# Jason9339/Wavelet-Noise-in-ray-tracing

Hardware: AMD Instinct MI355X
Metric: Mnoise-samples/sec (3D wavelet, octave=4) (higher is better)
Workload: dtype f32; 1 GPU; 512^3 dense 3D WNoise grid, tile=128, octave=4 (configs[1]); tile=128, seed=12345, octave=4, device=AMD Radeon Graphics (gfx950:sramecc+:xnack-)

## Files before the change

### wavelet-noise-in-ray-tracing_amd/csrc/wn_wavelet_multiband.hip

```cpp
#include "wn_internal.hpp"

#include <algorithm>
#include <cmath>
#include <type_traits>

namespace {

using wn::GridArgs;

typedef float v4f __attribute__((ext_vector_type(4)));
typedef float v2f __attribute__((ext_vector_type(2)));

constexpr int kMaxNB = 5;
constexpr int kWW = 8, kPW = 4, kSW = 4;
constexpr int kWaves = kWW + kPW + kSW;
constexpr int kPasses = 2 * kPW;
constexpr int kBX = 512, kBY = 8, kBZ = 8;
constexpr int kRing = 4;
constexpr int kSlotZ = 8, kSlotX = 16;
constexpr int kMaxK = 5;
constexpr int kRRow = kPasses * 64;
constexpr int kRPlane = kBY * kRRow;
constexpr int kRingFloats = kRing * kBY * kBX;
constexpr int kBoxFloats = 6144;
constexpr int kDmaPlanes = kMaxNB;
constexpr int kDmaLanded = kBZ - 2;

struct MbBand {
    float oscale;
    float factor;
    int first_pass;
    int K;
    int box_off;
    int rowlen;
};

struct MbArgs {
    const float *coef;
    float *out;
    int n, nmask;
    GridArgs g;
    float inv_den;
    int nbx, nby, nbz;
    int all_full;
    MbBand band[kMaxNB];
    int pass_band[kPasses];
};

__device__ __forceinline__ float readlane_f(float v, int l)
{
    return __int_as_float(__builtin_amdgcn_readlane(__float_as_int(v), l));
}

template <int NB>
__global__ __launch_bounds__(64 * kWaves) void grid3d_mbp_kernel(const MbArgs a)
{
    extern __shared__ __attribute__((aligned(16))) float lds[];
    __shared__ __attribute__((aligned(16))) float s_box[kBoxFloats];
    __shared__ int s_mid[3][NB][32];
    __shared__ float s_w[3][NB][kSlotX][3];
    __shared__ float s_oscale[NB];
    __shared__ __attribute__((aligned(16))) float s_wy[NB][kMaxK][kBY];
    __shared__ float s_wz[NB][64];
    __shared__ int s_prep[NB][4];
    __shared__ int s_bandc[NB][4];

    const int tid = threadIdx.x, lane = tid & 63;
    const int wave = __builtin_amdgcn_readfirstlane(tid >> 6);
    const bool is_window = wave < kWW, is_collapse = wave >= kWW && wave < kWW + kPW;
    const GridArgs &g = a.g;
    float *const ring = lds + 2 * kRPlane;

    const int nyz = a.nby * a.nbz;
    const long long total = (long long)a.nbx * nyz;
    const int item0 = (int)(total * blockIdx.x / gridDim.x), item1 = (int)(total * (blockIdx.x + 1) / gridDim.x);
    const int nb = item1 - item0;
    if (nb <= 0) return;
    const int G = nb * kBZ;

    struct Brick { int bx, by, bz; };
    auto brick_of = [&](int item) {
        Brick k;
        k.bx = item / nyz;
        k.by = (item - k.bx * nyz) / a.nbz;
        k.bz = item - k.bx * nyz - k.by * a.nbz;
        return k;
    };
    auto advance = [&](Brick &k) {
        if (++k.bz == a.nbz) { k.bz = 0; ++k.by; }
        if (k.by == a.nby) { k.by = 0; ++k.bx; }
    };

    auto fill_tables = [&](int buf, const Brick &k) {
        int tt = tid;
        asm volatile("" : "+v"(tt));
        const int b = tt >> 5, slot = tt & 31;
        if (b < NB && slot < kSlotX + 2) {
            int idx;
            if (slot < kSlotZ) idx = min(k.by * kBY + slot, g.ny - 1);
            else if (slot < kSlotX) idx = g.z0 + min(k.bz * kBZ + slot - kSlotZ, g.nz - 1);
            else idx = (slot == kSlotX) ? k.bx * kBX : min(k.bx * kBX + kBX - 1, g.nx - 1);
            const float c = wn::lattice_coord_fast(idx, (float)g.den, a.inv_den, g.base_range, s_oscale[b], g.post_scale);
            int m;
            float w0, w1, w2;
            wn::bspline(c, m, w0, w1, w2);
            s_mid[buf][b][slot] = m;
            if (slot < kSlotX) {
                s_w[buf][b][slot][0] = w0;
                s_w[buf][b][slot][1] = w1;
                s_w[buf][b][slot][2] = w2;
            }
        }
    };
    auto sgpr = [](int v) { return __builtin_amdgcn_readfirstlane(v); };
    auto fresh_rows = [&](int b, int K, int tA, int tB, bool same_column) {
        const int d = sgpr(s_mid[tB][b][kSlotZ]) - sgpr(s_mid[tA][b][kSlotZ]);
        return (same_column && d >= 0 && d <= 2) ? d : K;
    };

    auto derive_tables = [&](int b, int tA, int tB, bool same_column, bool first) {
        const int l = lane;
        {
            const int K = s_bandc[b][0];
            const int kz0 = s_mid[tB][b][kSlotZ] - 1;
            const int kzm = (K == 4) ? (kz0 & 3) : ((kz0 + 20 * 65536) % 5);
            {
                const int zi = l >> 3, j = l & 7;
                int t0 = kzm + (s_mid[tB][b][kSlotZ + zi] - s_mid[tB][b][kSlotZ]);
                t0 -= (t0 >= K) ? K : 0;
                const float w0 = s_w[tB][b][kSlotZ + zi][0], w1 = s_w[tB][b][kSlotZ + zi][1], w2 = s_w[tB][b][kSlotZ + zi][2];
                s_wz[b][l] = j == 0 ? w0 : j == 1 ? w1 : j == 2 ? w2 : __int_as_float(t0);
            }
            if (l < kMaxK * kBY) {
                const int j = l >> 3, yi = l & 7;
                const int dd = j - (s_mid[tB][b][yi] - s_mid[tB][b][0]);
                const float w0 = s_w[tB][b][yi][0], w1 = s_w[tB][b][yi][1], w2 = s_w[tB][b][yi][2];
                float f = a.band[0].factor;
#pragma unroll
                for (int bb = 1; bb < NB; ++bb) f = (b == bb) ? a.band[bb].factor : f;
                s_wy[b][j][yi] = ((unsigned)dd <= 2u ? (dd == 0 ? w0 : dd == 1 ? w1 : w2) : 0.0f) * f;
            }
            if (l == 0) {
                const int dz = s_mid[tB][b][kSlotZ] - s_mid[tA][b][kSlotZ];
                s_prep[b][0] = kzm;
                s_prep[b][1] = (!first && same_column && dz >= 0 && dz <= 2) ? dz : K;
                s_prep[b][2] = (s_mid[tB][b][kSlotX] - 1) & 3;
            }
        }
    };

    Brick cur = brick_of(item0), nxt = cur;
    advance(nxt);
    Brick nxt2 = nxt;
    advance(nxt2);
    if (tid < NB) {
        int K = a.band[0].K, box_off = a.band[0].box_off, rowlen = a.band[0].rowlen, fp = a.band[0].first_pass;
#pragma unroll
        for (int bb = 1; bb < NB; ++bb) {
            K = (tid == bb) ? a.band[bb].K : K;
            box_off = (tid == bb) ? a.band[bb].box_off : box_off;
            rowlen = (tid == bb) ? a.band[bb].rowlen : rowlen;
            fp = (tid == bb) ? a.band[bb].first_pass : fp;
        }
        s_bandc[tid][0] = K;
        s_bandc[tid][1] = box_off;
        s_bandc[tid][2] = rowlen;
        s_bandc[tid][3] = fp;
        float os = a.band[0].oscale;
#pragma unroll
        for (int bb = 1; bb < NB; ++bb) os = (tid == bb) ? a.band[bb].oscale : os;
        s_oscale[tid] = os;
    }
    __syncthreads();
    fill_tables(0, cur);
    if (nb > 1) fill_tables(1, nxt);
    __syncthreads();
    int tb = 0, t = 0;
    auto next_brick = [&]() {
        cur = nxt;
        nxt = nxt2;
        advance(nxt2);
        tb = (tb == 2) ? 0 : tb + 1;
        ++t;
    };

    if (is_collapse) {
        struct Pass {
            int id, band, col0, box_off, rowlen;
            float factor;
        };
        Pass ps[2];
        int pk[2];
#pragma unroll
        for (int i = 0; i < 2; ++i) {
            Pass &P = ps[i];
            P.id = (wave - kWW) + kPW * i;
            P.band = sgpr(a.pass_band[P.id]);
            const int bb0 = max(P.band, 0);
            pk[i] = P.band >= 0 ? sgpr(s_bandc[bb0][0]) : 0;
            P.box_off = sgpr(s_bandc[bb0][1]);
            P.rowlen = sgpr(s_bandc[bb0][2]);
            P.col0 = 64 * (P.id - sgpr(s_bandc[bb0][3]));
            float f = a.band[0].factor;
#pragma unroll
            for (int bb = 1; bb < NB; ++bb) f = (bb0 == bb) ? a.band[bb].factor : f;
            P.factor = __int_as_float(sgpr(__float_as_int(f)));
        }
        auto prep_brick = [&](const Pass &P, auto &yc, float &wzv, auto kc) {
            constexpr int K = decltype(kc)::value;
            if constexpr (K > 0) {
                const int kzm = sgpr(s_prep[P.band][0]), d = sgpr(s_prep[P.band][1]);
                wzv = s_wz[P.band][lane];
                const float *img = s_box + P.box_off + min(sgpr(s_prep[P.band][2]) + P.col0 + lane, P.rowlen - 1);
#pragma unroll
                for (int sl = 0; sl < K; ++sl) {
                    const int tau = (sl - kzm + K) % K;
                    if (tau >= K - d) {
                        const float *row = img + (tau - (K - d)) * K * P.rowlen;
#pragma unroll
                        for (int j = 0; j < K; ++j) {
                            const float cj = row[j * P.rowlen];
                            const v2f c2 = {cj, cj};
#pragma unroll
                            for (int h = 0; h < 2; ++h) {
                                const v4f w4 = *reinterpret_cast<const v4f *>(&s_wy[P.band][j][4 * h]);
                                const v2f wlo = {w4.x, w4.y}, whi = {w4.z, w4.w};
                                yc[2 * h][sl] = (j == 0) ? wlo * c2 : __builtin_elementwise_fma(wlo, c2, yc[2 * h][sl]);
                                yc[2 * h + 1][sl] = (j == 0) ? whi * c2 : __builtin_elementwise_fma(whi, c2, yc[2 * h + 1][sl]);
                            }
                        }
                    }
                }
            }
        };
        auto p1_slice = [&](float *Rw, int zi, const auto &yc, float wzv, auto kc) {
            constexpr int K = decltype(kc)::value;
            if constexpr (K > 0) {
                const float w0 = readlane_f(wzv, zi * 8), w1 = readlane_f(wzv, zi * 8 + 1), w2 = readlane_f(wzv, zi * 8 + 2);
                const int t0 = __builtin_amdgcn_readlane(__float_as_int(wzv), zi * 8 + 3);
                auto taps = [&](auto tc) {
                    constexpr int T0 = decltype(tc)::value, T1 = (T0 + 1) % K, T2 = (T0 + 2) % K;
#pragma unroll
                    for (int p2 = 0; p2 < kBY / 2; ++p2) {
                        v2f v = v2f{w0, w0} * yc[p2][T0];
                        v = __builtin_elementwise_fma(v2f{w1, w1}, yc[p2][T1], v);
                        v = __builtin_elementwise_fma(v2f{w2, w2}, yc[p2][T2], v);
                        Rw[(2 * p2) * kRRow] = v.x;
                        Rw[(2 * p2 + 1) * kRRow] = v.y;
                    }
                };
                using std::integral_constant;
                if (t0 == 0) taps(integral_constant<int, 0>{});
                else if (t0 == 1) taps(integral_constant<int, 1>{});
                else if (t0 == 2) taps(integral_constant<int, 2>{});
                else if (t0 == 3 || K == 4) taps(integral_constant<int, 3>{});
                else taps(integral_constant<int, K - 1>{});
            }
        };
        auto collapse_role = [&](auto k0c, auto k1c) {
            constexpr int K0 = decltype(k0c)::value, K1 = decltype(k1c)::value;
            v2f yc0[kBY / 2][K0 > 0 ? K0 : 1], yc1[kBY / 2][K1 > 0 ? K1 : 1];
            float wzv0 = 0.0f, wzv1 = 0.0f;
            float *const Rw0 = lds + 64 * ps[0].id + lane, *const Rw1 = lds + 64 * ps[1].id + lane;
            wn::lds_barrier();
            prep_brick(ps[0], yc0, wzv0, k0c);
            prep_brick(ps[1], yc1, wzv1, k1c);
            p1_slice(Rw0, 0, yc0, wzv0, k0c);
            p1_slice(Rw1, 0, yc1, wzv1, k1c);
            wn::lds_barrier();
            for (int gp = 0; gp < G + 2; ++gp) {
                const int zi = gp & (kBZ - 1);
                if (gp < G) {
                    if (gp + 1 < G) {
                        if (zi == kBZ - 1) {
                            prep_brick(ps[0], yc0, wzv0, k0c);
                            prep_brick(ps[1], yc1, wzv1, k1c);
                        }
                        const int rs = ((gp + 1) & 1) * kRPlane;
                        p1_slice(Rw0 + rs, (gp + 1) & (kBZ - 1), yc0, wzv0, k0c);
                        p1_slice(Rw1 + rs, (gp + 1) & (kBZ - 1), yc1, wzv1, k1c);
                    }
                    if (zi == kBZ - 1) next_brick();
                }
                wn::lds_barrier();
            }
        };
        using std::integral_constant;
        const int k0 = pk[0], k1 = pk[1];
        if (k0 == 4 && k1 == 4) collapse_role(integral_constant<int, 4>{}, integral_constant<int, 4>{});
        else if (k0 == 4 && k1 == 5) collapse_role(integral_constant<int, 4>{}, integral_constant<int, 5>{});
        else if (k0 == 5 && k1 == 4) collapse_role(integral_constant<int, 5>{}, integral_constant<int, 4>{});
        else if (k0 == 5 && k1 == 5) collapse_role(integral_constant<int, 5>{}, integral_constant<int, 5>{});
        else if (k0 == 4) collapse_role(integral_constant<int, 4>{}, integral_constant<int, 0>{});
        else if (k0 == 5) collapse_role(integral_constant<int, 5>{}, integral_constant<int, 0>{});
        else collapse_role(integral_constant<int, 0>{}, integral_constant<int, 0>{});
    } else if (is_window) {
        const int xw = (wave >> 2) & 1, wr = wave & 3;
        float ww[NB][4][4];
        int wbase[NB];
        auto x_weights = [&](int tbuf, int bx) {
            const float den = (float)g.den;
            const int x0 = bx * kBX + xw * 256 + lane * 4;
            float xbase[4];
#pragma unroll
            for (int q = 0; q < 4; ++q) {
                const float xi = (float)min(x0 + q, g.nx - 1);
                xbase[q] = ((a.inv_den != 0.0f) ? xi * a.inv_den : xi / den) * g.base_range;
            }
#pragma unroll
            for (int b = 0; b < NB; ++b) {
                int m[4];
                float w[4][3];
#pragma unroll
                for (int q = 0; q < 4; ++q) {
                    float cc = xbase[q] * a.band[b].oscale;
                    cc = cc * g.post_scale;
                    wn::bspline(cc, m[q], w[q][0], w[q][1], w[q][2]);
                }
                wbase[b] = 64 * a.band[b].first_pass + m[0] - s_mid[tbuf][b][kSlotX];
#pragma unroll
                for (int q = 0; q < 4; ++q) {
                    const bool up = m[q] != m[0];
                    ww[b][q][0] = up ? 0.0f : w[q][0];
                    ww[b][q][1] = up ? w[q][0] : w[q][1];
                    ww[b][q][2] = up ? w[q][1] : w[q][2];
                    ww[b][q][3] = up ? w[q][2] : 0.0f;
                }
            }
        };
        auto phaseC = [&](int rslot, int ringslot) {
            float acc[2][4];
            const float *Rp = lds + rslot * kRPlane + wr * kRRow;
#pragma unroll
            for (int b = 0; b < NB; ++b) {
                float v[2][4];
#pragma unroll
                for (int h = 0; h < 2; ++h)
#pragma unroll
                    for (int i = 0; i < 4; ++i) v[h][i] = Rp[h * 4 * kRRow + wbase[b] + i];
#pragma unroll
                for (int h = 0; h < 2; ++h)
#pragma unroll
                    for (int q = 0; q < 4; ++q) {
                        float s = (b == 0) ? ww[b][q][0] * v[h][0] : __builtin_fmaf(ww[b][q][0], v[h][0], acc[h][q]);
                        s = __builtin_fmaf(ww[b][q][1], v[h][1], s);
                        s = __builtin_fmaf(ww[b][q][2], v[h][2], s);
                        s = __builtin_fmaf(ww[b][q][3], v[h][3], s);
                        acc[h][q] = s;
                    }
            }
#pragma unroll
            for (int h = 0; h < 2; ++h)
                *reinterpret_cast<v4f *>(ring + (ringslot * kBY + wr + 4 * h) * kBX + xw * 256 + lane * 4) =
                    v4f{acc[h][0], acc[h][1], acc[h][2], acc[h][3]};
        };

        x_weights(0, cur.bx);
        wn::lds_barrier();
        wn::lds_barrier();
        for (int gp = 0; gp < G + 2; ++gp) {
            const int zi = gp & (kBZ - 1);
            if (gp < G) {
                phaseC(gp & 1, gp & (kRing - 1));
                if (zi == kBZ - 1) {
                    const int tb1 = (tb == 2) ? 0 : tb + 1, tb2 = (tb1 == 2) ? 0 : tb1 + 1;
                    if (t + 2 < nb) fill_tables(tb2, nxt2);
                    if (t + 1 < nb && nxt.bx != cur.bx) x_weights(tb1, nxt.bx);
                    next_brick();
                }
            }
            wn::lds_barrier();
        }
    } else {
        const int sw = wave - (kWW + kPW);
        int bK[NB], bBox[NB], bRow[NB];
#pragma unroll
        for (int b = 0; b < NB; ++b) {
            bK[b] = sgpr(s_bandc[b][0]);
            bBox[b] = sgpr(s_bandc[b][1]);
            bRow[b] = sgpr(s_bandc[b][2]);
        }
        auto request_band = [&](auto bc, int tA, int tB, bool same_column, bool first) {
            constexpr int b = decltype(bc)::value;
            if constexpr (b < NB) {
                const int K = bK[b];
                const int d = first ? K : fresh_rows(b, K, tA, tB, same_column);
                const int jy0 = sgpr(s_mid[tB][b][0]) - 1, kz0 = sgpr(s_mid[tB][b][kSlotZ]) - 1 + (K - d);
                const int r = min(lane, K * K - 1);
                const int f = (K == 4) ? (r >> 2) : ((r * 13) >> 6);
                const int j = r - f * K;
                const int rowoff = (((kz0 + f) & a.nmask) * a.n + ((jy0 + j) & a.nmask)) * a.n;
                const int ix0 = (sgpr(s_mid[tB][b][kSlotX]) - 1) & ~3;
                const unsigned voff = (unsigned)((ix0 + 4 * lane) & a.nmask) * 4u;
                for (int rr = sw; rr < d * K; rr += kSW) {
                    const char *rowp = reinterpret_cast<const char *>(a.coef + __builtin_amdgcn_readlane(rowoff, rr));
                    if (4 * lane < bRow[b])
                        __builtin_amdgcn_global_load_lds((const __attribute__((address_space(1))) void *)(rowp + voff),
                                                         (__attribute__((address_space(3))) void *)&s_box[bBox[b] + rr * bRow[b]],
                                                         16, 0, 0);
                }
            }
        };
        Brick sb = cur;
        const size_t plane_stride = (size_t)g.ny * g.nx;
        float *orow = nullptr;
        auto brick_pointer = [&]() {
            orow = a.out + ((size_t)(sb.bz * kBZ) * g.ny + sb.by * kBY + 2 * sw) * g.nx + sb.bx * kBX + lane * 4;
        };
        brick_pointer();
        auto store_plane = [&](int p) {
            const int zi = p & (kBZ - 1), ringslot = p & (kRing - 1);
            const float *src = ring + (ringslot * kBY + 2 * sw) * kBX + lane * 4;
            v4f v[4];
#pragma unroll
            for (int q = 0; q < 4; ++q) v[q] = *reinterpret_cast<const v4f *>(src + (q >> 1) * kBX + (q & 1) * 256);
            if (a.all_full) {
#pragma unroll
                for (int q = 0; q < 4; ++q) *reinterpret_cast<v4f *>(orow + (size_t)(q >> 1) * g.nx + (q & 1) * 256) = v[q];
            } else {
                const int z = sb.bz * kBZ + zi;
#pragma unroll
                for (int q = 0; q < 4; ++q) {
                    const int row = 2 * sw + (q >> 1), xh = q & 1;
                    const int y = sb.by * kBY + row, x = sb.bx * kBX + xh * 256 + lane * 4;
                    if (y < g.ny && z < g.nz && x + 3 < g.nx)
                        *reinterpret_cast<v4f *>(orow + (size_t)(q >> 1) * g.nx + (q & 1) * 256) = v[q];
                }
            }
            orow += plane_stride;
            if (zi == kBZ - 1) {
                advance(sb);
                brick_pointer();
            }
        };

        using std::integral_constant;
        request_band(integral_constant<int, 0>{}, 0, 0, false, true);
        request_band(integral_constant<int, 1>{}, 0, 0, false, true);
        request_band(integral_constant<int, 2>{}, 0, 0, false, true);
        request_band(integral_constant<int, 3>{}, 0, 0, false, true);
        request_band(integral_constant<int, 4>{}, 0, 0, false, true);
        for (int b = sw; b < NB; b += kSW) derive_tables(b, 0, 0, false, true);
        asm volatile("s_waitcnt vmcnt(0)" ::: "memory");
        wn::lds_barrier();
        wn::lds_barrier();
        for (int gp = 0; gp < G + 2; ++gp) {
            const int zi = gp & (kBZ - 1);
            if (gp >= 2) store_plane(gp - 2);
            if (gp < G) {
                if (zi < NB && t + 1 < nb) {
                    const int tb1 = (tb == 2) ? 0 : tb + 1;
                    const bool same = nxt.bx == cur.bx && nxt.by == cur.by;
                    if (zi == 0) request_band(integral_constant<int, 0>{}, tb, tb1, same, false);
                    else if (zi == 1) request_band(integral_constant<int, 1>{}, tb, tb1, same, false);
                    else if (zi == 2) request_band(integral_constant<int, 2>{}, tb, tb1, same, false);
                    else if (zi == 3) request_band(integral_constant<int, 3>{}, tb, tb1, same, false);
                    else request_band(integral_constant<int, 4>{}, tb, tb1, same, false);
                }
                if (zi == kBZ - 2 && t + 1 < nb)
                    for (int b = sw; b < NB; b += kSW)
                        derive_tables(b, tb, (tb == 2) ? 0 : tb + 1, nxt.bx == cur.bx && nxt.by == cur.by, false);
                if (zi == kDmaLanded) {
                    if (a.all_full) asm volatile("s_waitcnt vmcnt(%0)" ::"n"(4 * (kDmaLanded - kDmaPlanes + 1)) : "memory");
                    else asm volatile("s_waitcnt vmcnt(0)" ::: "memory");
                }
                if (zi == kBZ - 1) next_brick();
            }
            wn::lds_barrier();
        }
    }
}

template <int NB>
bool launch_mbp(const MbArgs &a, size_t lds, long long bricks, hipStream_t s)
{
    const void *fn = reinterpret_cast<const void *>(&grid3d_mbp_kernel<NB>);
    if (!wn::ensure_dynamic_lds(fn, wn::current_device(), lds)) return false;
    const int cus = wn::device_compute_units(wn::current_device());
    const int grid = (int)std::min<long long>(bricks, cus);
    hipLaunchKernelGGL((grid3d_mbp_kernel<NB>), dim3(grid), dim3(64 * kWaves), lds, s, a);
    return true;
}

}

namespace wn {

int multiband_try(const wn_tile *tile, const GridArgs &g, int nbands, const float *oscale, const float *weights,
                  float out_div, float *out_dev, hipStream_t stream, int min_bricks_per_cu)
{
    if (nbands < 1 || nbands > kMaxNB || tile->n == 0 || wn::pow2_mask(tile->n) < 0) return kDeclined;
    if (g.nx <= 256 || !vec4_ok(out_dev, g.nx) || g.ny <= 0 || g.nz <= 0 || g.z_const_mode || g.z0 < 0) return kDeclined;
    MbArgs a{};
    int passes = 0, box_off = 0;
    for (int w = 0; w < kPasses; ++w) a.pass_band[w] = -1;
    for (int b = 0; b < nbands; ++b) {
        LatticeStep ls;
        if (!lattice_step(g, oscale[b], false, false, 0.0, &ls) || !ls.two_mids()) return kDeclined;
        const int K = (int)std::max<long long>(4, std::max(ls.extent(kBY), ls.extent(kBZ)));
        if (K > kMaxK) return kDeclined;
        const int ex = (int)ls.extent(kBX) + 1;
        const int np = (ex + 63) / 64;
        if (passes + np > kPasses) return kDeclined;
        a.band[b].first_pass = passes;
        for (int p = 0; p < np; ++p) a.pass_band[passes++] = b;
        a.band[b].oscale = oscale[b];
        a.band[b].factor = (float)((double)(weights ? weights[b] : 1.0f) * (double)g.out_scale / (double)out_div);
        a.band[b].K = K;
        a.band[b].rowlen = (ex + 3 + 3) & ~3;
        if (a.band[b].rowlen > 256) return kDeclined;
        a.band[b].box_off = box_off;
        box_off += K * K * a.band[b].rowlen;
    }
    if (box_off > kBoxFloats) return kDeclined;
    const size_t lds = (size_t)(2 * kRPlane + kRingFloats) * sizeof(float);
    a.coef = tile->dev;
    a.out = out_dev;
    a.n = tile->n;
    a.nmask = wn::pow2_mask(tile->n);
    a.g = g;
    a.inv_den = wn::inv_den_of(g.den);
    a.nbx = (g.nx + kBX - 1) / kBX;
    a.nby = (g.ny + kBY - 1) / kBY;
    a.nbz = (g.nz + kBZ - 1) / kBZ;
    a.all_full = (g.nx % kBX == 0 && g.ny % kBY == 0 && g.nz % kBZ == 0) ? 1 : 0;
    const long long bricks = (long long)a.nbx * a.nby * a.nbz;
    if (bricks > 0x7fffffffLL / kBZ) return kDeclined;
    if (bricks < (long long)min_bricks_per_cu * wn::device_compute_units(wn::current_device())) return kDeclined;
    if ((long long)a.nbx * kBX * 10 > (long long)g.nx * 11) return kDeclined;
    bool ok;
    switch (nbands) {
    case 1: ok = launch_mbp<1>(a, lds, bricks, stream); break;
    case 2: ok = launch_mbp<2>(a, lds, bricks, stream); break;
    case 3: ok = launch_mbp<3>(a, lds, bricks, stream); break;
    case 4: ok = launch_mbp<4>(a, lds, bricks, stream); break;
    default: ok = launch_mbp<5>(a, lds, bricks, stream); break;
    }
    if (!ok) return kDeclined;
    WN_LAUNCH_CHECK("grid3d_mbp_kernel");
    return WN_OK;
}

}
```

Measured before the change: 1.395 million Msamples/s.

## Batch-plan per-brick z/y/x weight tables into a ring ahead of use

Replaces the per-brick fill_tables/derive_tables path with a plan_pass that precomputes z-weights, DMA prep values, and per-column y-weights and x mids for up to 16 bricks at once into LDS ring buffers. The store waves do this planning only when a new column or block starts, and the window waves stop doing table fills. Kernel arguments are copied into SGPR-pinned locals and global pointers get an explicit address space, so loads use the global path. The initial DMA requests move into a prologue on the store waves. The cost is extra LDS for the plan rings and a more complex slot/column-buffer indexing scheme.

```diff
diff --git a/wavelet-noise-in-ray-tracing_amd/csrc/wn_wavelet_multiband.hip b/wavelet-noise-in-ray-tracing_amd/csrc/wn_wavelet_multiband.hip
--- a/wavelet-noise-in-ray-tracing_amd/csrc/wn_wavelet_multiband.hip
+++ b/wavelet-noise-in-ray-tracing_amd/csrc/wn_wavelet_multiband.hip
@@ -10,6 +10,8 @@
 
 typedef float v4f __attribute__((ext_vector_type(4)));
 typedef float v2f __attribute__((ext_vector_type(2)));
+typedef __attribute__((address_space(1))) float gfloat;
+typedef __attribute__((address_space(1))) v4f gv4f;
 
 constexpr int kMaxNB = 5;
 constexpr int kWW = 8, kPW = 4, kSW = 4;
@@ -17,7 +19,8 @@
 constexpr int kPasses = 2 * kPW;
 constexpr int kBX = 512, kBY = 8, kBZ = 8;
 constexpr int kRing = 4;
-constexpr int kSlotZ = 8, kSlotX = 16;
+constexpr int kPlanBricks = 16;
+constexpr int kPlanRing = 2 * kPlanBricks;
 constexpr int kMaxK = 5;
 constexpr int kRRow = kPasses * 64;
 constexpr int kRPlane = kBY * kRRow;
@@ -53,22 +56,34 @@
 }
 
 template <int NB>
-__global__ __launch_bounds__(64 * kWaves) void grid3d_mbp_kernel(const MbArgs a)
+__global__ __launch_bounds__(64 * kWaves) void grid3d_mbp_kernel(const MbArgs args)
 {
     extern __shared__ __attribute__((aligned(16))) float lds[];
     __shared__ __attribute__((aligned(16))) float s_box[kBoxFloats];
-    __shared__ int s_mid[3][NB][32];
-    __shared__ float s_w[3][NB][kSlotX][3];
-    __shared__ float s_oscale[NB];
-    __shared__ __attribute__((aligned(16))) float s_wy[NB][kMaxK][kBY];
-    __shared__ float s_wz[NB][64];
-    __shared__ int s_prep[NB][4];
     __shared__ int s_bandc[NB][4];
+    __shared__ float s_oscale[NB], s_factor[NB];
+    __shared__ int s_passband[kPasses];
+    __shared__ v4f s_pz[kPlanRing][NB][kBZ];
+    __shared__ __attribute__((aligned(16))) int s_pprep[kPlanRing][NB][4];
+    __shared__ __attribute__((aligned(16))) float s_wy[2][NB][kMaxK][kBY];
+    __shared__ int s_pcol[2][NB][2];
 
     const int tid = threadIdx.x, lane = tid & 63;
     const int wave = __builtin_amdgcn_readfirstlane(tid >> 6);
     const bool is_window = wave < kWW, is_collapse = wave >= kWW && wave < kWW + kPW;
-    const GridArgs &g = a.g;
+    struct {
+        const gfloat *coef;
+        gfloat *out;
+        int n, nmask, nbx, nby, nbz, all_full;
+        float inv_den;
+    } a = {(const gfloat *)args.coef, (gfloat *)args.out, args.n, args.nmask, args.nbx, args.nby, args.nbz, args.all_full, args.inv_den};
+    struct {
+        int den, nx, ny, z0, nz;
+        float base_range, post_scale;
+    } g = {args.g.den, args.g.nx, args.g.ny, args.g.z0, args.g.nz, args.g.base_range, args.g.post_scale};
+    asm volatile("" : "+s"(a.coef), "+s"(a.out), "+s"(a.n), "+s"(a.nmask), "+s"(a.nbx), "+s"(a.nby), "+s"(a.nbz), "+s"(a.all_full),
+                 "+s"(a.inv_den));
+    asm volatile("" : "+s"(g.den), "+s"(g.nx), "+s"(g.ny), "+s"(g.z0), "+s"(g.nz), "+s"(g.base_range), "+s"(g.post_scale));
     float *const ring = lds + 2 * kRPlane;
 
     const int nyz = a.nby * a.nbz;
@@ -90,61 +105,77 @@
         if (++k.bz == a.nbz) { k.bz = 0; ++k.by; }
         if (k.by == a.nby) { k.by = 0; ++k.bx; }
     };
-
-    auto fill_tables = [&](int buf, const Brick &k) {
-        int tt = tid;
+    auto same_column = [](const Brick &p, const Brick &q) { return p.bx == q.bx && p.by == q.by; };
+    auto sgpr = [](int v) { return __builtin_amdgcn_readfirstlane(v); };
+
+    auto sample = [&](int idx, float os, int &m, float &w0, float &w1, float &w2) {
+        const float c = wn::lattice_coord_fast(idx, (float)g.den, a.inv_den, g.base_range, os, g.post_scale);
+        wn::bspline(c, m, w0, w1, w2);
+    };
+    auto y_index = [&](int by, int yi) { return min(by * kBY + yi, g.ny - 1); };
+    auto z_index = [&](int bz, int zi) { return g.z0 + min(bz * kBZ + zi, g.nz - 1); };
+    auto x_index = [&](int bx) { return bx * kBX; };
+
+    auto request_rows = [&](int sw, int K, int box, int rowlen, int d, int kzf, int jy0, int ixm) {
+        const int r = min(lane, K * K - 1);
+        const int f = (K == 4) ? (r >> 2) : ((r * 13) >> 6);
+        const int j = r - f * K;
+        const int rowoff = (((kzf + f) & a.nmask) * a.n + ((jy0 + j) & a.nmask)) * a.n;
+        const int ix0 = ixm & ~3;
+        const unsigned voff = (unsigned)((ix0 + 4 * lane) & a.nmask) * 4u;
+        for (int rr = sw; rr < d * K; rr += kSW) {
+            const gfloat *rowp = a.coef + __builtin_amdgcn_readlane(rowoff, rr);
+            if (4 * lane < rowlen)
+                __builtin_amdgcn_global_load_lds((const __attribute__((address_space(1))) void *)(rowp + voff / 4u),
+                                                 (__attribute__((address_space(3))) void *)&s_box[box + rr * rowlen], 16, 0, 0);
+        }
+    };
+
+    auto plan_pass = [&](int i0, int stride, int t0, const Brick &k0, int L, bool cont, int colbuf) {
+        int tt = i0;
         asm volatile("" : "+v"(tt));
-        const int b = tt >> 5, slot = tt & 31;
-        if (b < NB && slot < kSlotX + 2) {
-            int idx;
-            if (slot < kSlotZ) idx = min(k.by * kBY + slot, g.ny - 1);
-            else if (slot < kSlotX) idx = g.z0 + min(k.bz * kBZ + slot - kSlotZ, g.nz - 1);
-            else idx = (slot == kSlotX) ? k.bx * kBX : min(k.bx * kBX + kBX - 1, g.nx - 1);
-            const float c = wn::lattice_coord_fast(idx, (float)g.den, a.inv_den, g.base_range, s_oscale[b], g.post_scale);
-            int m;
-            float w0, w1, w2;
-            wn::bspline(c, m, w0, w1, w2);
-            s_mid[buf][b][slot] = m;
-            if (slot < kSlotX) {
-                s_w[buf][b][slot][0] = w0;
-                s_w[buf][b][slot][1] = w1;
-                s_w[buf][b][slot][2] = w2;
-            }
-        }
-    };
-    auto sgpr = [](int v) { return __builtin_amdgcn_readfirstlane(v); };
-    auto fresh_rows = [&](int b, int K, int tA, int tB, bool same_column) {
-        const int d = sgpr(s_mid[tB][b][kSlotZ]) - sgpr(s_mid[tA][b][kSlotZ]);
-        return (same_column && d >= 0 && d <= 2) ? d : K;
-    };
-
-    auto derive_tables = [&](int b, int tA, int tB, bool same_column, bool first) {
-        const int l = lane;
-        {
-            const int K = s_bandc[b][0];
-            const int kz0 = s_mid[tB][b][kSlotZ] - 1;
-            const int kzm = (K == 4) ? (kz0 & 3) : ((kz0 + 20 * 65536) % 5);
-            {
-                const int zi = l >> 3, j = l & 7;
-                int t0 = kzm + (s_mid[tB][b][kSlotZ + zi] - s_mid[tB][b][kSlotZ]);
-                t0 -= (t0 >= K) ? K : 0;
-                const float w0 = s_w[tB][b][kSlotZ + zi][0], w1 = s_w[tB][b][kSlotZ + zi][1], w2 = s_w[tB][b][kSlotZ + zi][2];
-                s_wz[b][l] = j == 0 ? w0 : j == 1 ? w1 : j == 2 ? w2 : __int_as_float(t0);
-            }
-            if (l < kMaxK * kBY) {
-                const int j = l >> 3, yi = l & 7;
-                const int dd = j - (s_mid[tB][b][yi] - s_mid[tB][b][0]);
-                const float w0 = s_w[tB][b][yi][0], w1 = s_w[tB][b][yi][1], w2 = s_w[tB][b][yi][2];
-                float f = a.band[0].factor;
-#pragma unroll
-                for (int bb = 1; bb < NB; ++bb) f = (b == bb) ? a.band[bb].factor : f;
-                s_wy[b][j][yi] = ((unsigned)dd <= 2u ? (dd == 0 ? w0 : dd == 1 ? w1 : w2) : 0.0f) * f;
-            }
-            if (l == 0) {
-                const int dz = s_mid[tB][b][kSlotZ] - s_mid[tA][b][kSlotZ];
-                s_prep[b][0] = kzm;
-                s_prep[b][1] = (!first && same_column && dz >= 0 && dz <= 2) ? dz : K;
-                s_prep[b][2] = (s_mid[tB][b][kSlotX] - 1) & 3;
+        const int nzi = L * (NB * kBZ);
+        const int items = nzi + (colbuf >= 0 ? NB * (kMaxK * kBY + 1) : 0);
+        for (int i = tt; i < items; i += stride) {
+            float u0, u1, u2, w0, w1, w2;
+            if (i < nzi) {
+                const int zi = i & (kBZ - 1), cb = i >> 3, c = cb / NB, b = cb - c * NB;
+                const int K = s_bandc[b][0];
+                const float os = s_oscale[b];
+                const int bz = k0.bz + c;
+                int m0, m;
+                sample(z_index(bz, 0), os, m0, u0, u1, u2);
+                sample(z_index(bz, zi), os, m, w0, w1, w2);
+                const int kz0 = m0 - 1;
+                const int kzm = (K == 4) ? (kz0 & 3) : ((kz0 + 20 * 65536) % 5);
+                int tp = kzm + (m - m0);
+                tp -= (tp >= K) ? K : 0;
+                const int slot = (t0 + c) & (kPlanRing - 1);
+                s_pz[slot][b][zi] = v4f{w0, w1, w2, __int_as_float(tp)};
+                if (zi == 0) {
+                    int mp;
+                    sample(z_index(bz - 1, 0), os, mp, u0, u1, u2);
+                    const int dz = m0 - mp;
+                    const int d = ((c > 0 || cont) && dz >= 0 && dz <= 2) ? dz : K;
+                    s_pprep[slot][b][0] = kzm;
+                    s_pprep[slot][b][1] = d;
+                    s_pprep[slot][b][2] = kz0 + (K - d);
+                }
+            } else {
+                const int q = i - nzi, b = q / (kMaxK * kBY + 1), l = q - b * (kMaxK * kBY + 1);
+                const float os = s_oscale[b];
+                int m0, m;
+                sample(y_index(k0.by, 0), os, m0, u0, u1, u2);
+                if (l < kMaxK * kBY) {
+                    const int j = l >> 3, yi = l & 7;
+                    sample(y_index(k0.by, yi), os, m, w0, w1, w2);
+                    const int dd = j - (m - m0);
+                    s_wy[colbuf][b][j][yi] = ((unsigned)dd <= 2u ? (dd == 0 ? w0 : dd == 1 ? w1 : w2) : 0.0f) * s_factor[b];
+                } else {
+                    sample(x_index(k0.bx), os, m, w0, w1, w2);
+                    s_pcol[colbuf][b][0] = m0 - 1;
+                    s_pcol[colbuf][b][1] = m;
+                }
             }
         }
     };
@@ -154,40 +185,73 @@
     Brick nxt2 = nxt;
     advance(nxt2);
     if (tid < NB) {
-        int K = a.band[0].K, box_off = a.band[0].box_off, rowlen = a.band[0].rowlen, fp = a.band[0].first_pass;
+        int K = args.band[0].K, box_off = args.band[0].box_off, rowlen = args.band[0].rowlen, fp = args.band[0].first_pass;
+        float os = args.band[0].oscale, f = args.band[0].factor;
 #pragma unroll
         for (int bb = 1; bb < NB; ++bb) {
-            K = (tid == bb) ? a.band[bb].K : K;
-            box_off = (tid == bb) ? a.band[bb].box_off : box_off;
-            rowlen = (tid == bb) ? a.band[bb].rowlen : rowlen;
-            fp = (tid == bb) ? a.band[bb].first_pass : fp;
+            K = (tid == bb) ? args.band[bb].K : K;
+            box_off = (tid == bb) ? args.band[bb].box_off : box_off;
+            rowlen = (tid == bb) ? args.band[bb].rowlen : rowlen;
+            fp = (tid == bb) ? args.band[bb].first_pass : fp;
+            os = (tid == bb) ? args.band[bb].oscale : os;
+            f = (tid == bb) ? args.band[bb].factor : f;
         }
         s_bandc[tid][0] = K;
         s_bandc[tid][1] = box_off;
         s_bandc[tid][2] = rowlen;
         s_bandc[tid][3] = fp;
-        float os = a.band[0].oscale;
-#pragma unroll
-        for (int bb = 1; bb < NB; ++bb) os = (tid == bb) ? a.band[bb].oscale : os;
         s_oscale[tid] = os;
+        s_factor[tid] = f;
     }
-    __syncthreads();
-    fill_tables(0, cur);
-    if (nb > 1) fill_tables(1, nxt);
-    __syncthreads();
-    int tb = 0, t = 0;
+    if (tid < kPasses) {
+        int pb = args.pass_band[0];
+#pragma unroll
+        for (int w = 1; w < kPasses; ++w) pb = (tid == w) ? args.pass_band[w] : pb;
+        s_passband[tid] = pb;
+    }
+    if (!is_window && !is_collapse) {
+        float os[NB];
+        int bK[NB], bBox[NB], bRow[NB];
+#pragma unroll
+        for (int b = 0; b < NB; ++b) {
+            os[b] = args.band[b].oscale;
+            bK[b] = args.band[b].K;
+            bBox[b] = args.band[b].box_off;
+            bRow[b] = args.band[b].rowlen;
+        }
+#pragma unroll
+        for (int b = 0; b < NB; ++b) asm volatile("" : "+s"(os[b]), "+s"(bK[b]), "+s"(bBox[b]), "+s"(bRow[b]));
+        const int axis = lane & 3;
+        const int idx = axis == 0 ? y_index(cur.by, 0) : axis == 1 ? z_index(cur.bz, 0) : x_index(cur.bx);
+        float osl = os[0];
+#pragma unroll
+        for (int b = 1; b < NB; ++b) osl = ((lane >> 2) == b) ? os[b] : osl;
+        int m;
+        float w0, w1, w2;
+        sample(idx, osl, m, w0, w1, w2);
+#pragma unroll
+        for (int b = 0; b < NB; ++b)
+            request_rows(wave - (kWW + kPW), bK[b], bBox[b], bRow[b], bK[b], __builtin_amdgcn_readlane(m, 4 * b + 1) - 1,
+                         __builtin_amdgcn_readlane(m, 4 * b) - 1, __builtin_amdgcn_readlane(m, 4 * b + 2) - 1);
+    }
+    wn::lds_barrier();
+    const bool column1 = nb > 1 && !same_column(cur, nxt);
+    plan_pass(tid, 64 * kWaves, 0, cur, min(min(kPlanBricks, a.nbz - cur.bz), nb), false, 0);
+    if (column1) plan_pass(tid, 64 * kWaves, 1, nxt, min(min(kPlanBricks - 1, a.nbz - nxt.bz), nb - 1), false, 1);
+    wn::lds_barrier();
+    int t = 0;
+    int cbn = column1 ? 1 : 0;
     auto next_brick = [&]() {
+        cbn ^= same_column(nxt, nxt2) ? 0 : 1;
         cur = nxt;
         nxt = nxt2;
         advance(nxt2);
-        tb = (tb == 2) ? 0 : tb + 1;
         ++t;
     };
 
     if (is_collapse) {
         struct Pass {
             int id, band, col0, box_off, rowlen;
-            float factor;
         };
         Pass ps[2];
         int pk[2];
@@ -195,23 +259,19 @@
         for (int i = 0; i < 2; ++i) {
             Pass &P = ps[i];
             P.id = (wave - kWW) + kPW * i;
-            P.band = sgpr(a.pass_band[P.id]);
+            P.band = sgpr(s_passband[P.id]);
             const int bb0 = max(P.band, 0);
             pk[i] = P.band >= 0 ? sgpr(s_bandc[bb0][0]) : 0;
             P.box_off = sgpr(s_bandc[bb0][1]);
             P.rowlen = sgpr(s_bandc[bb0][2]);
             P.col0 = 64 * (P.id - sgpr(s_bandc[bb0][3]));
-            float f = a.band[0].factor;
-#pragma unroll
-            for (int bb = 1; bb < NB; ++bb) f = (bb0 == bb) ? a.band[bb].factor : f;
-            P.factor = __int_as_float(sgpr(__float_as_int(f)));
-        }
-        auto prep_brick = [&](const Pass &P, auto &yc, float &wzv, auto kc) {
+        }
+        auto prep_brick = [&](const Pass &P, auto &yc, float &wzv, auto kc, int slot, int cb) {
             constexpr int K = decltype(kc)::value;
             if constexpr (K > 0) {
-                const int kzm = sgpr(s_prep[P.band][0]), d = sgpr(s_prep[P.band][1]);
-                wzv = s_wz[P.band][lane];
-                const float *img = s_box + P.box_off + min(sgpr(s_prep[P.band][2]) + P.col0 + lane, P.rowlen - 1);
+                const int kzm = sgpr(s_pprep[slot][P.band][0]), d = sgpr(s_pprep[slot][P.band][1]);
+                wzv = reinterpret_cast<const float *>(&s_pz[slot][P.band][0])[(lane >> 3) * 4 + (lane & 3)];
+                const float *img = s_box + P.box_off + min(((sgpr(s_pcol[cb][P.band][1]) - 1) & 3) + P.col0 + lane, P.rowlen - 1);
 #pragma unroll
                 for (int sl = 0; sl < K; ++sl) {
                     const int tau = (sl - kzm + K) % K;
@@ -223,7 +283,7 @@
                             const v2f c2 = {cj, cj};
 #pragma unroll
                             for (int h = 0; h < 2; ++h) {
-                                const v4f w4 = *reinterpret_cast<const v4f *>(&s_wy[P.band][j][4 * h]);
+                                const v4f w4 = *reinterpret_cast<const v4f *>(&s_wy[cb][P.band][j][4 * h]);
                                 const v2f wlo = {w4.x, w4.y}, whi = {w4.z, w4.w};
                                 yc[2 * h][sl] = (j == 0) ? wlo * c2 : __builtin_elementwise_fma(wlo, c2, yc[2 * h][sl]);
                                 yc[2 * h + 1][sl] = (j == 0) ? whi * c2 : __builtin_elementwise_fma(whi, c2, yc[2 * h + 1][sl]);
@@ -263,8 +323,8 @@
             float wzv0 = 0.0f, wzv1 = 0.0f;
             float *const Rw0 = lds + 64 * ps[0].id + lane, *const Rw1 = lds + 64 * ps[1].id + lane;
             wn::lds_barrier();
-            prep_brick(ps[0], yc0, wzv0, k0c);
-            prep_brick(ps[1], yc1, wzv1, k1c);
+            prep_brick(ps[0], yc0, wzv0, k0c, 0, 0);
+            prep_brick(ps[1], yc1, wzv1, k1c, 0, 0);
             p1_slice(Rw0, 0, yc0, wzv0, k0c);
             p1_slice(Rw1, 0, yc1, wzv1, k1c);
             wn::lds_barrier();
@@ -273,8 +333,9 @@
                 if (gp < G) {
                     if (gp + 1 < G) {
                         if (zi == kBZ - 1) {
-                            prep_brick(ps[0], yc0, wzv0, k0c);
-                            prep_brick(ps[1], yc1, wzv1, k1c);
+                            const int slot = (t + 1) & (kPlanRing - 1);
+                            prep_brick(ps[0], yc0, wzv0, k0c, slot, cbn);
+                            prep_brick(ps[1], yc1, wzv1, k1c, slot, cbn);
                         }
                         const int rs = ((gp + 1) & 1) * kRPlane;
                         p1_slice(Rw0 + rs, (gp + 1) & (kBZ - 1), yc0, wzv0, k0c);
@@ -298,7 +359,7 @@
         const int xw = (wave >> 2) & 1, wr = wave & 3;
         float ww[NB][4][4];
         int wbase[NB];
-        auto x_weights = [&](int tbuf, int bx) {
+        auto x_weights = [&](int cb, int bx) {
             const float den = (float)g.den;
             const int x0 = bx * kBX + xw * 256 + lane * 4;
             float xbase[4];
@@ -311,13 +372,14 @@
             for (int b = 0; b < NB; ++b) {
                 int m[4];
                 float w[4][3];
+                const float os = s_oscale[b];
 #pragma unroll
                 for (int q = 0; q < 4; ++q) {
-                    float cc = xbase[q] * a.band[b].oscale;
+                    float cc = xbase[q] * os;
                     cc = cc * g.post_scale;
                     wn::bspline(cc, m[q], w[q][0], w[q][1], w[q][2]);
                 }
-                wbase[b] = 64 * a.band[b].first_pass + m[0] - s_mid[tbuf][b][kSlotX];
+                wbase[b] = 64 * s_bandc[b][3] + m[0] - s_pcol[cb][b][1];
 #pragma unroll
                 for (int q = 0; q < 4; ++q) {
                     const bool up = m[q] != m[0];
@@ -363,9 +425,7 @@
             if (gp < G) {
                 phaseC(gp & 1, gp & (kRing - 1));
                 if (zi == kBZ - 1) {
-                    const int tb1 = (tb == 2) ? 0 : tb + 1, tb2 = (tb1 == 2) ? 0 : tb1 + 1;
-                    if (t + 2 < nb) fill_tables(tb2, nxt2);
-                    if (t + 1 < nb && nxt.bx != cur.bx) x_weights(tb1, nxt.bx);
+                    if (t + 1 < nb && nxt.bx != cur.bx) x_weights(cbn, nxt.bx);
                     next_brick();
                 }
             }
@@ -380,30 +440,17 @@
             bBox[b] = sgpr(s_bandc[b][1]);
             bRow[b] = sgpr(s_bandc[b][2]);
         }
-        auto request_band = [&](auto bc, int tA, int tB, bool same_column, bool first) {
+        auto request_band = [&](auto bc) {
             constexpr int b = decltype(bc)::value;
             if constexpr (b < NB) {
-                const int K = bK[b];
-                const int d = first ? K : fresh_rows(b, K, tA, tB, same_column);
-                const int jy0 = sgpr(s_mid[tB][b][0]) - 1, kz0 = sgpr(s_mid[tB][b][kSlotZ]) - 1 + (K - d);
-                const int r = min(lane, K * K - 1);
-                const int f = (K == 4) ? (r >> 2) : ((r * 13) >> 6);
-                const int j = r - f * K;
-                const int rowoff = (((kz0 + f) & a.nmask) * a.n + ((jy0 + j) & a.nmask)) * a.n;
-                const int ix0 = (sgpr(s_mid[tB][b][kSlotX]) - 1) & ~3;
-                const unsigned voff = (unsigned)((ix0 + 4 * lane) & a.nmask) * 4u;
-                for (int rr = sw; rr < d * K; rr += kSW) {
-                    const char *rowp = reinterpret_cast<const char *>(a.coef + __builtin_amdgcn_readlane(rowoff, rr));
-                    if (4 * lane < bRow[b])
-                        __builtin_amdgcn_global_load_lds((const __attribute__((address_space(1))) void *)(rowp + voff),
-                                                         (__attribute__((address_space(3))) void *)&s_box[bBox[b] + rr * bRow[b]],
-                                                         16, 0, 0);
-                }
+                const int slot = (t + 1) & (kPlanRing - 1);
+                request_rows(sw, bK[b], bBox[b], bRow[b], sgpr(s_pprep[slot][b][1]), sgpr(s_pprep[slot][b][2]),
+                             sgpr(s_pcol[cbn][b][0]), sgpr(s_pcol[cbn][b][1]) - 1);
             }
         };
         Brick sb = cur;
         const size_t plane_stride = (size_t)g.ny * g.nx;
-        float *orow = nullptr;
+        gfloat *orow = nullptr;
         auto brick_pointer = [&]() {
             orow = a.out + ((size_t)(sb.bz * kBZ) * g.ny + sb.by * kBY + 2 * sw) * g.nx + sb.bx * kBX + lane * 4;
         };
@@ -416,7 +463,7 @@
             for (int q = 0; q < 4; ++q) v[q] = *reinterpret_cast<const v4f *>(src + (q >> 1) * kBX + (q & 1) * 256);
             if (a.all_full) {
 #pragma unroll
-                for (int q = 0; q < 4; ++q) *reinterpret_cast<v4f *>(orow + (size_t)(q >> 1) * g.nx + (q & 1) * 256) = v[q];
+                for (int q = 0; q < 4; ++q) *reinterpret_cast<gv4f *>(orow + (size_t)(q >> 1) * g.nx + (q & 1) * 256) = v[q];
             } else {
                 const int z = sb.bz * kBZ + zi;
 #pragma unroll
@@ -424,7 +471,7 @@
                     const int row = 2 * sw + (q >> 1), xh = q & 1;
                     const int y = sb.by * kBY + row, x = sb.bx * kBX + xh * 256 + lane * 4;
                     if (y < g.ny && z < g.nz && x + 3 < g.nx)
-                        *reinterpret_cast<v4f *>(orow + (size_t)(q >> 1) * g.nx + (q & 1) * 256) = v[q];
+                        *reinterpret_cast<gv4f *>(orow + (size_t)(q >> 1) * g.nx + (q & 1) * 256) = v[q];
                 }
             }
             orow += plane_stride;
@@ -435,12 +482,6 @@
         };
 
         using std::integral_constant;
-        request_band(integral_constant<int, 0>{}, 0, 0, false, true);
-        request_band(integral_constant<int, 1>{}, 0, 0, false, true);
-        request_band(integral_constant<int, 2>{}, 0, 0, false, true);
-        request_band(integral_constant<int, 3>{}, 0, 0, false, true);
-        request_band(integral_constant<int, 4>{}, 0, 0, false, true);
-        for (int b = sw; b < NB; b += kSW) derive_tables(b, 0, 0, false, true);
         asm volatile("s_waitcnt vmcnt(0)" ::: "memory");
         wn::lds_barrier();
         wn::lds_barrier();
@@ -449,22 +490,26 @@
             if (gp >= 2) store_plane(gp - 2);
             if (gp < G) {
                 if (zi < NB && t + 1 < nb) {
-                    const int tb1 = (tb == 2) ? 0 : tb + 1;
-                    const bool same = nxt.bx == cur.bx && nxt.by == cur.by;
-                    if (zi == 0) request_band(integral_constant<int, 0>{}, tb, tb1, same, false);
-                    else if (zi == 1) request_band(integral_constant<int, 1>{}, tb, tb1, same, false);
-                    else if (zi == 2) request_band(integral_constant<int, 2>{}, tb, tb1, same, false);
-                    else if (zi == 3) request_band(integral_constant<int, 3>{}, tb, tb1, same, false);
-                    else request_band(integral_constant<int, 4>{}, tb, tb1, same, false);
-                }
-                if (zi == kBZ - 2 && t + 1 < nb)
-                    for (int b = sw; b < NB; b += kSW)
-                        derive_tables(b, tb, (tb == 2) ? 0 : tb + 1, nxt.bx == cur.bx && nxt.by == cur.by, false);
+                    if (zi == 0) request_band(integral_constant<int, 0>{});
+                    else if (zi == 1) request_band(integral_constant<int, 1>{});
+                    else if (zi == 2) request_band(integral_constant<int, 2>{});
+                    else if (zi == 3) request_band(integral_constant<int, 3>{});
+                    else request_band(integral_constant<int, 4>{});
+                }
                 if (zi == kDmaLanded) {
                     if (a.all_full) asm volatile("s_waitcnt vmcnt(%0)" ::"n"(4 * (kDmaLanded - kDmaPlanes + 1)) : "memory");
                     else asm volatile("s_waitcnt vmcnt(0)" ::: "memory");
                 }
-                if (zi == kBZ - 1) next_brick();
+                if (zi == kBZ - 1) {
+                    if (t + 2 < nb) {
+                        const bool cont = same_column(nxt, nxt2);
+                        const int left = kPlanBricks - ((t + 2) & (kPlanBricks - 1));
+                        if (!cont || left == kPlanBricks)
+                            plan_pass(tid - 64 * (kWW + kPW), 64 * kSW, t + 2, nxt2, min(min(left, a.nbz - nxt2.bz), nb - (t + 2)),
+                                      cont, cont ? -1 : (cbn ^ 1));
+                    }
+                    next_brick();
+                }
             }
             wn::lds_barrier();
         }
```

Result: no change. 1.392 million Msamples/s, median of 2 (-0.2%).
